# Tonz24/restir-embree

Measured on AMD Instinct MI355X. Metric: Mrays/s + frames/s at 1080p, 32 candidates, 4 spatial neighbours, higher is better.
Workload: dtype f32; 1 GPU; C2: Cornell box + 1024 emissive 0.02 m quads, A=32 B=1, spatial k=4 P=1 R=30 CONSTANT MIS, temporal off, cap 20, 1920x1080; width=1920, height=1080, traversal=lockstep, frames_in_flight=3, wide_tree=668, parallelism=1 GPU

## Files before the change

### restir-embree_amd/csrc/rs_passes.h

```cpp
#pragma once
#include "rs_scene.h"
#include "rs_texture.h"

#ifndef RS_INITIAL_WAVES
#define RS_INITIAL_WAVES 5
#endif
#ifndef RS_SPATIAL_WAVES
#define RS_SPATIAL_WAVES 4
#endif
#ifndef RS_SPATIAL_WAVES_SMALL
#define RS_SPATIAL_WAVES_SMALL 5
#endif
#ifndef RS_INITIAL_WAVES_LANE
#define RS_INITIAL_WAVES_LANE 6
#endif
#ifndef RS_SPATIAL_WAVES_LANE
#define RS_SPATIAL_WAVES_LANE 5
#endif
#ifndef RS_TEMPORAL_WAVES
#define RS_TEMPORAL_WAVES 4
#endif
#ifndef RS_TEMPORAL_WAVES_LANE
#define RS_TEMPORAL_WAVES_LANE 5
#endif
#define RS_WAVES(T, lockstep, lane) (((T) & TRAV_LANE) ? (lane) : (lockstep))
#ifndef RS_RIS_BATCH
#define RS_RIS_BATCH 2
#endif
#ifndef RS_RIS_BATCH_LANE
#define RS_RIS_BATCH_LANE 1
#endif

namespace rs {

struct FrameConst {
    int m_area, m_brdf, k, spatial_passes, cap;
    float radius, min_normal_sim, max_depth_diff;
    int do_spatial, do_temporal, do_vis_pass, reject, mis;
    vec3 bg; float tnear_off, tfar_off, normal_off;
    int use_sky;
    uint32_t seed, frame;
    int W, H;
    int y0, y1;
    int gy0, gy1;
    float inv_view[9];
    float inv_view_prev[9];
    GCam cam, camp;
    const int* row_order;
    int n_order;
    int debug_reproj;
    int canon_vis;
    uint8_t* dbg;
    float* cand_w;
    float4* cand_ray;
};

struct Counters { unsigned long long rays, primary, reproj_outside; };

struct CountSlot {
    uint2* part;
    unsigned long long* outside;
    float* row_cost;
    int y0, y1;
};

__device__ __forceinline__ uint32_t wave_sum(uint32_t v) {
    for (int o = 32; o > 0; o >>= 1) v += __shfl_xor(v, o, 64);
    return v;
}
__device__ __forceinline__ uint64_t wave_clock() { return __builtin_amdgcn_s_memrealtime(); }
__device__ __forceinline__ void row_cost_add(CountSlot C, uint64_t t0, int y) {
    if (!C.row_cost) return;
    constexpr int kRows = 8;
    const int yt = __builtin_amdgcn_readfirstlane(y) + (int)(threadIdx.x & 63);
    const float w = (float)(wave_clock() - t0) * (1.0f / kRows);
    if ((threadIdx.x & 63) < kRows && yt >= C.y0 && yt < C.y1) atomicAdd(C.row_cost + yt, w);
}
__device__ __forceinline__ void count_rays(CountSlot C, uint32_t rays, uint32_t primary, uint64_t t0, int y) {
    uint32_t r = wave_sum(rays), p = wave_sum(primary);
    if ((threadIdx.x & 63) == 0)
        C.part[((size_t)blockIdx.y * gridDim.x + blockIdx.x) * (blockDim.x >> 6) + (threadIdx.x >> 6)] = make_uint2(r, p);
    row_cost_add(C, t0, y);
}

constexpr int kReduceBlocks = 128, kReduceThreads = 64;
__device__ __forceinline__ void block_sum2(unsigned long long& r, unsigned long long& p) {
    __shared__ unsigned long long sr[16], sp[16];
    for (int o = 32; o > 0; o >>= 1) { r += __shfl_xor(r, o, 64); p += __shfl_xor(p, o, 64); }
    const int w = threadIdx.x >> 6, nw = blockDim.x >> 6;
    if ((threadIdx.x & 63) == 0) { sr[w] = r; sp[w] = p; }
    __syncthreads();
    r = 0; p = 0;
    if (threadIdx.x == 0)
        for (int i = 0; i < nw; ++i) { r += sr[i]; p += sp[i]; }
}
__global__ void __launch_bounds__(kReduceThreads) k_reduce_counts(const uint2* part, size_t n, ulonglong2* partial,
                                                                  unsigned* ticket, Counters* out, Counters* tot) {
    const size_t chunk = (n + gridDim.x - 1) / gridDim.x, b = blockIdx.x * chunk, e = b + chunk < n ? b + chunk : n;
    unsigned long long r = 0, p = 0;
    for (size_t i = b + threadIdx.x; i < e; i += kReduceThreads) { uint2 v = part[i]; r += v.x; p += v.y; }
    block_sum2(r, p);
    __shared__ bool last;
    if (threadIdx.x == 0) {
        __hip_atomic_store(&partial[blockIdx.x].x, r, __ATOMIC_RELAXED, __HIP_MEMORY_SCOPE_AGENT);
        __hip_atomic_store(&partial[blockIdx.x].y, p, __ATOMIC_RELAXED, __HIP_MEMORY_SCOPE_AGENT);
        last = __hip_atomic_fetch_add(ticket, 1u, __ATOMIC_ACQ_REL, __HIP_MEMORY_SCOPE_AGENT) == gridDim.x - 1;
    }
    __syncthreads();
    if (!last) return;
    r = 0; p = 0;
    for (unsigned i = threadIdx.x; i < gridDim.x; i += kReduceThreads) {
        r += __hip_atomic_load(&partial[i].x, __ATOMIC_RELAXED, __HIP_MEMORY_SCOPE_AGENT);
        p += __hip_atomic_load(&partial[i].y, __ATOMIC_RELAXED, __HIP_MEMORY_SCOPE_AGENT);
    }
// ... 54 lines not shown
    float cI = gmax(dot(ld, sf.nrm), 0.0f);
    float cY = fabsf(dot(-ld, s.n));
    float G = cI * cY / r2;
    r.L = (s.li * eval_brdf<Call>(sf, ld)) * G;
    r.need = r.ok && test_vis && !(r.L.x == 0.0f && r.L.y == 0.0f && r.L.z == 0.0f);
    r.dir = ld;
    r.tfar = sqrtf(r2) - F.tfar_off;
    return r;
}
__device__ __forceinline__ FPre evaluate_f_pre(const FrameConst& F, const Sample& s, vec3 cam, const GElem& g,
                                               bool test_vis, bool alive) {
    return evaluate_f_pre(F, s, g.pos, g.le.x > 0 || g.le.y > 0 || g.le.z > 0, make_frame(g, cam), test_vis, alive);
}
__device__ __forceinline__ vec3 evaluate_f_post(const FPre& p, bool occ) {
    vec3 L = p.L;
    if (p.need) L = L * (float)(!occ);
    return p.ok ? L : mk(0, 0, 0);
}
template <int T>
__device__ __forceinline__ vec3 evaluate_f(const DevScene& S, const FrameConst& F, const Sample& s, vec3 pos,
                                           bool emissive, const ShadeFrame& sf, bool test_vis, bool alive,
                                           uint32_t& rays) {
    FPre p = evaluate_f_pre(F, s, pos, emissive, sf, test_vis, alive);
    bool occ = false;
    if (test_vis) {
        rays += p.need ? 1u : 0u;
        occ = trace_any<T>(S, p.need, pos, p.dir, FLT_MIN + F.tnear_off, p.tfar);
    }
    return evaluate_f_post(p, occ);
}
template <int T>
__device__ __forceinline__ vec3 evaluate_f(const DevScene& S, const FrameConst& F, const Sample& s, vec3 cam,
                                           const GElem& g, bool test_vis, bool alive, uint32_t& rays) {
    FPre p = evaluate_f_pre(F, s, cam, g, test_vis, alive);
    bool occ = false;
    if (test_vis) {
        rays += p.need ? 1u : 0u;
        occ = trace_any<T>(S, p.need, g.pos, p.dir, FLT_MIN + F.tnear_off, p.tfar);
    }
    return evaluate_f_post(p, occ);
}

__device__ __forceinline__ float m_area(const FrameConst& F, float pa, float pb) {
    if (pa == 0.0f && pb == 0.0f) return 0.0f;
    return pa / ((float)F.m_area * pa + (float)F.m_brdf * pb);
}
__device__ __forceinline__ float m_brdf(const FrameConst& F, float pb, float pa) {
    if (pa == 0.0f && pb == 0.0f) return 0.0f;
    return pb / ((float)F.m_area * pa + (float)F.m_brdf * pb);
}

template <int T>
__device__ __forceinline__ GElem gbuffer_fill_cam(const DevScene& S, const FrameConst& F, const GCam& cam,
                                                  const float* m, int x, int y, bool active) {
    vec3 dc = mk((float)x - (float)F.W / 2.0f, (float)F.H / 2.0f - (float)y, -cam.focal);
    vec3 dw = mk(m[0] * dc.x + m[3] * dc.y + m[6] * dc.z, m[1] * dc.x + m[4] * dc.y + m[7] * dc.z,
                 m[2] * dc.x + m[5] * dc.y + m[8] * dc.z);
    dw = normalize(dw);
    SurfHit h = intersect<T>(S, active, cam.pos, dw, FLT_MIN + 0.01f);
    GElem g;
    g.pos = mk(0, 0, 0); g.nrm = g.pos; g.kd = g.pos; g.ks = g.pos; g.le = g.pos;
    g.shin = 0; g.depth = 0; g.type = 0; g.inv_im = 0;
    if (h.hit) {
        MatRec mr = load_mat(S, h.mat);
        vec3 nrm = h.normal;
        if (S.texd) apply_maps(S, h, mr, nrm, false);
        g.pos = h.point; g.nrm = nrm; g.depth = length(h.point - cam.pos);
        g.type = mr.type; g.kd = mr.kd; g.ks = mr.ks; g.le = mr.le; g.shin = mr.shin;
        if (g.type == MT_PHONG || g.type == MT_DIELECTRIC) {
            vec3 V = normalize(cam.pos - g.pos);
            g.inv_im = 1.0f / calc_I_M(dot(V, g.nrm), g.shin);
        }
    } else {
        g.le = F.use_sky ? sky_texel(S, dw) : F.bg;
    }
    return g;
}
template <int T>
__device__ __forceinline__ GElem gbuffer_fill(const DevScene& S, const FrameConst& F, int x, int y, bool active) {
    return gbuffer_fill_cam<T>(S, F, F.cam, F.inv_view, x, y, active);
}

struct LightGlobal {
    const float* cdf_g;
    const int* guide_g;
    __device__ __forceinline__ explicit LightGlobal(const DevScene& S) : cdf_g(S.cdf), guide_g(S.cdf_guide) {}
    __device__ __forceinline__ float cdf(uint32_t i) const { return cdf_g[i]; }
    __device__ __forceinline__ uint32_t guide(uint32_t j) const { return (uint32_t)guide_g[j]; }
};
template <class LT>
__device__ __forceinline__ uint32_t light_index(const LT& L, uint32_t n_emis, float ksi) {
    uint32_t j = (uint32_t)(ksi * (float)kCdfGuide);
    uint32_t lo = L.guide(j), n = L.guide(j + 1) + 1u - lo;
    if (lo + n > n_emis) n = n_emis - lo;
    while (n > 0) {
        uint32_t h = n >> 1;
        if (L.cdf(lo + h) < ksi) { lo = lo + h + 1; n = n - h - 1; } else n = h;
    }
    return lo < n_emis ? lo : n_emis - 1;
}
__device__ __forceinline__ uint32_t light_index(const DevScene& S, float ksi) {
    return light_index(LightGlobal(S), S.n_emis, ksi);
}

constexpr int kLightLdsMax = 2048;
static_assert(kLightLdsMax <= 65535, "the LDS guide holds CDF indices as uint16_t");
static_assert(kLightLdsMax % 4 == 0 && kLightLdsMax / 4 == 2 * 256 && kCdfGuide == 4 * 256,
              "LightFill: a 256-thread workgroup moves the CDF as 2 and the guide as 1 16-B load per thread");
constexpr int LIGHT_LDS = 8;
struct LightLds {
    const float* cdf_l;
    const uint16_t* guide_l;
    __device__ __forceinline__ float cdf(uint32_t i) const { return cdf_l[i]; }
    __device__ __forceinline__ uint32_t guide(uint32_t j) const { return (uint32_t)guide_l[j]; }
};
struct LightFill {
    float4 c[2];
    int4 g;
    int g_end;
    __device__ __forceinline__ static float4 cdf4(const float* cdf, uint32_t i, uint32_t n) {
        if (4u * i + 4u <= n) return reinterpret_cast<const float4*>(cdf)[i];
        float4 v = make_float4(1.0f, 1.0f, 1.0f, 1.0f);
        if (4u * i < n) v.x = cdf[4u * i];
        if (4u * i + 1u < n) v.y = cdf[4u * i + 1u];
        if (4u * i + 2u < n) v.z = cdf[4u * i + 2u];
        return v;
    }
    __device__ __forceinline__ void issue(const DevScene& S, uint32_t t) {
        const uint32_t n = S.n_emis < (uint32_t)kLightLdsMax ? S.n_emis : (uint32_t)kLightLdsMax;
        c[0] = cdf4(S.cdf, t, n);
        c[1] = cdf4(S.cdf, t + 256u, n);
        g = reinterpret_cast<const int4*>(S.cdf_guide)[t];
        g_end = t == 0 ? S.cdf_guide[kCdfGuide] : 0;
    }
    __device__ __forceinline__ void commit(float* cdf_l, uint16_t* guide_l, uint32_t t) const {
        float4* c4 = reinterpret_cast<float4*>(cdf_l);
        uint2* g2 = reinterpret_cast<uint2*>(guide_l);
        c4[t] = c[0];
        c4[t + 256u] = c[1];
        g2[t] = make_uint2((uint32_t)g.x | ((uint32_t)g.y << 16), (uint32_t)g.z | ((uint32_t)g.w << 16));
        if (t == 0) guide_l[kCdfGuide] = (uint16_t)g_end;
    }
};

template <class LT>
__device__ __forceinline__ uint32_t area_pick(const LT& L, const DevScene& S, const Rng& rng, int c) {
    Rng q = rng;
    q.n = cand_slot(c);
    return light_index(L, S.n_emis, q.range(0.0f, 1.0f));
}
__device__ __forceinline__ uint32_t area_pick(const DevScene& S, const Rng& rng, int c) {
    return area_pick(LightGlobal(S), S, rng, c);
}
struct EmisRec {
    vec3 p0, p1, p2, n0, n1, n2, le;
    float pdf_area;
    __device__ __forceinline__ static EmisRec load(const float4* E) {
        const float4 a = E[0], b = E[1], c = E[2], d = E[3];
        EmisRec r;
        r.p0 = xyz(a); r.p1 = xyz(b); r.p2 = xyz(c); r.le = xyz(d);
        r.n0 = mk(b.w, c.w, d.w);
        r.n1 = r.n0; r.n2 = r.n0;
        if (__float_as_uint(a.w) >> 31) { r.n1 = xyz(E[4]); r.n2 = xyz(E[5]); }
        r.pdf_area = fabsf(a.w);
        return r;
    }
};
__device__ __forceinline__ float emis_pdf_brdf(const DevScene& S, int id) { return S.emis[8 * id + 5].w; }

template <bool Call = false>
__device__ __forceinline__ Sample area_sample_at(const DevScene& S, const FrameConst& F, vec3 pos, const ShadeFrame& sf,
                                                 Rng& rng, uint32_t idx, float& W_out, float& mis_out) {
    const EmisRec E = EmisRec::load(S.emis + 8 * idx);
    float r1 = rng.range(0, 1), r2 = rng.range(0, 1);
    float sr = sqrtf(r1);
    float bx = 1.0f - sr, by = sr * (1.0f - r2), bz = sr * r2;
    vec3 pt = (E.p0 * bx + E.p1 * by) + E.p2 * bz;
    vec3 nn = normalize((E.n0 * bx + E.n1 * by) + E.n2 * bz);
    float pdf_area = E.pdf_area;
    vec3 ld = pt - pos;
    float r2s = dot(ld, ld);
    ld = normalize(ld);
    float cY = gmax(dot(-ld, nn), 0.0f);
    float amf = cY / r2s;
    float pba = phong_pdf<Call>(sf, ld) * amf;
    mis_out = m_area(F, pdf_area, pba);
    W_out = 1.0f / pdf_area;
    return Sample{pt, nn, E.le};
}
template <class LT>
__device__ __forceinline__ Sample area_sample(const LT& L, const DevScene& S, const FrameConst& F, vec3 pos,
                                              const ShadeFrame& sf, Rng& rng, float& W_out, float& mis_out) {
    const uint32_t idx = light_index(L, S.n_emis, rng.range(0.0f, 1.0f));
    return area_sample_at(S, F, pos, sf, rng, idx, W_out, mis_out);
}

template <int T>
__device__ __forceinline__ Sample brdf_sample(const DevScene& S, const FrameConst& F, vec3 pos, const ShadeFrame& sf,
                                              bool alive, Rng& rng, float& W_out, float& mis_out, uint32_t& rays) {
    float pdf;
    vec3 wi = sample_brdf(sf, rng, pdf);
    vec3 org = pos + sf.nrm * F.normal_off;
    rays += alive ? 1u : 0u;
    SurfHit h = intersect<T | TRAV_LANE>(S, alive, org, wi, FLT_MIN + F.tnear_off);
    W_out = 0.0f; mis_out = 0.0f;
    if (h.hit) {
        MatRec mr = load_mat(S, h.mat);
        if (mr.le.x + mr.le.y + mr.le.z > 0) {
            vec3 hn = h.normal;
            if (S.texd) apply_maps(S, h, mr, hn, true);
            vec3 ld = h.point - pos;
            float r2s = dot(ld, ld);
            ld = normalize(ld);
            float cY = gmax(dot(-ld, hn), 0.0f);
            float amf = cY / r2s;
            float pdf_area = emis_pdf_brdf(S, h.emis_id);
            float bpa = pdf * amf;
            W_out = 1.0f / bpa;
            mis_out = m_brdf(F, bpa, pdf_area);
            return Sample{h.point, hn, mr.le};
        }
    }
    return smp_invalid();
}

struct FrameSlot {
    float4* base;
    int t, n;
    __device__ __forceinline__ void store(const ShadeFrame& s) const {
        base[t] = f4(s.nrm, s.pf);
        base[n + t] = f4(s.wr, s.omp);
        base[2 * n + t] = f4(s.kd_pi, s.shin);
        base[3 * n + t] = f4(s.ks_im, s.a);
        base[4 * n + t] = make_float4(s.maxD, s.maxS, __int_as_float(s.type), 0.0f);
    }
    __device__ __forceinline__ ShadeFrame load() const {
        asm volatile("" ::: "memory");
        const float4 a = base[t], b = base[n + t], c = base[2 * n + t], d = base[3 * n + t], e = base[4 * n + t];
        ShadeFrame s;
        s.nrm = xyz(a); s.pf = a.w; s.wr = xyz(b); s.omp = b.w; s.kd_pi = xyz(c); s.shin = c.w;
        s.ks_im = xyz(d); s.a = d.w; s.maxD = e.x; s.maxS = e.y; s.type = __float_as_int(e.z);
        return s;
    }
};

template <int T, int kB>
__device__ __forceinline__ void area_batch(const DevScene& S, const FrameConst& F, vec3 pos, const ShadeFrame& sf,
                                           Rng& rng, int c0, int c_end, bool alive, bool tv, const uint32_t* pick,
                                           float* w_out, uint32_t& rays) {
    float wu[kB], wo[kB];
    bool act[kB], okb[kB], occ[kB];
    vec3 dir[kB];
    float tf[kB];
    const float inv_ma = 1.0f / (float)F.m_area;
#pragma unroll
    for (int k = 0; k < kB; ++k) {
        float Wc, mis;
        rng.n = cand_slot(c0 + k) + 1u;
        const Sample s = area_sample_at(S, F, pos, sf, rng, pick[k], Wc, mis);
        const FPre p = evaluate_f_pre(F, s, pos, false, sf, tv, alive && c0 + k < c_end);
        const float ph = length(p.L);
        const float m = F.m_brdf > 0 ? mis : inv_ma;
        wu[k] = m * ph * Wc;
        wo[k] = m * 0.0f * Wc;
        act[k] = p.need; okb[k] = p.ok; dir[k] = p.dir; tf[k] = p.tfar; occ[k] = false;
        rays += act[k] ? 1u : 0u;
    }
    if (tv) trace_any_multi<T, kB>(S, act, pos, dir, FLT_MIN + F.tnear_off, tf, occ);
#pragma unroll
    for (int k = 0; k < kB; ++k) w_out[k] = (okb[k] && !(act[k] && occ[k])) ? wu[k] : wo[k];
}
template <class LT>
__device__ __forceinline__ Sample area_redraw(const LT& L, const DevScene& S, const FrameConst& F, vec3 pos,
                                             const ShadeFrame& sf, Rng& rng, int c, bool tv, vec3& f) {
    float Wc, mis;
    rng.n = cand_slot(c);
    const Sample s = area_sample(L, S, F, pos, sf, rng, Wc, mis);
    f = evaluate_f_pre(F, s, pos, false, sf, tv, true).L;
    return s;
}
__device__ __forceinline__ Sample area_redraw(const DevScene& S, const FrameConst& F, vec3 pos, const ShadeFrame& sf,
                                             Rng& rng, int c, bool tv, vec3& f) {
    return area_redraw(LightGlobal(S), S, F, pos, sf, rng, c, tv, f);
}

template <int T, class LT>
__device__ __forceinline__ Res initial_ris(const LT& L, const DevScene& S, const FrameConst& F, vec3 pos, bool emissive,
                                           FrameSlot fs, uint32_t pix, bool in_pass, vec3& f_sel, uint32_t& rays) {
    f_sel = mk(0, 0, 0);
    Res r = res_empty();
    const bool alive = in_pass && !emissive && S.n_emis > 0;
    if (__ballot(alive) == 0) return r;
    Rng rng; rng.init(F.seed, F.frame, PASS_INITIAL, pix);
    const bool tv = !F.do_vis_pass;
    constexpr int kB = trav_lane(T) ? RS_RIS_BATCH_LANE : RS_RIS_BATCH;
    float best_phat = 0.0f;
    if (F.m_area > 0) {
        int sel = -1;
        uint32_t pick[kB];
#pragma unroll
        for (int k = 0; k < kB; ++k) pick[k] = area_pick(L, S, rng, k);
        for (int c0 = 0; c0 < F.m_area; c0 += kB) {
            float w[kB];
            uint32_t next[kB];
#pragma unroll
            for (int k = 0; k < kB; ++k) next[k] = area_pick(L, S, rng, c0 + kB + k);
            area_batch<T, kB>(S, F, pos, fs.load(), rng, c0, F.m_area, alive, tv, pick, w, rays);
#pragma unroll
            for (int k = 0; k < kB; ++k) pick[k] = next[k];
#pragma unroll
            for (int k = 0; k < kB; ++k) {
                if (c0 + k < F.m_area) {
                    rng.n = cand_slot(c0 + k) + 3u;
                    if (alive && res_add_w(r, w[k], 0, rng)) sel = c0 + k;
                }
            }
        }
        if (sel >= 0) {
            const Sample s = area_redraw(L, S, F, pos, fs.load(), rng, sel, tv, f_sel);
            best_phat = length(f_sel);
            r.p = s.p; r.n = s.n; r.li = s.li;
        }
    }
    if (F.m_brdf > 0) {
        float inv_mb = 1.0f / (float)F.m_brdf;
        for (int i = 0; i < F.m_brdf; ++i) {
            float Wc, mis;
            rng.n = cand_slot(F.m_area + i);
            const ShadeFrame sf = fs.load();
            Sample s = brdf_sample<T>(S, F, pos, sf, alive, rng, Wc, mis, rays);
            vec3 f = evaluate_f<T>(S, F, s, pos, false, sf, tv, alive, rays);
            float ph = length(f);
            float w = F.m_area > 0 ? mis * ph * Wc : inv_mb * ph * Wc;
            rng.n = cand_slot(F.m_area + i) + 3u;
            if (alive && res_add(r, s, w, 0, rng)) { best_phat = ph; f_sel = f; }
        }
    }
    if (!alive) { f_sel = mk(0, 0, 0); return res_empty(); }
    r.conf = F.m_area + F.m_brdf;
    float ph = smp_valid(smp_of(r)) ? best_phat : 0.0f;
    r.W = ph > 0.0f ? 1.0f / ph * r.wsum : 0.0f;
    res_cap(r, F.cap);
    return r;
}

__device__ __forceinline__ vec3 shade_px(const Res& r, vec3 f, vec3 le) {
    vec3 px = r.wsum > 0.0f ? f * r.W : le;
    return sanitize(px);
}
__device__ __forceinline__ void store_rgb(float* fb, size_t p, vec3 c) {
    fb[3 * p] = c.x; fb[3 * p + 1] = c.y; fb[3 * p + 2] = c.z;
}

struct TileQ { uint32_t* ctr; uint32_t n; };
__device__ __forceinline__ uint32_t q_pull(const TileQ& Q) {
    uint32_t t = 0u;
    if ((threadIdx.x & 63) == 0) t = atomicAdd(Q.ctr, 1u);
    return (uint32_t)__builtin_amdgcn_readfirstlane((int)t);
}
__device__ __forceinline__ void q_exit(const TileQ& Q) {
    if ((threadIdx.x & 63) != 0) return;
    const uint32_t waves = gridDim.x * gridDim.y * (blockDim.x >> 6);
    if (__hip_atomic_fetch_add(Q.ctr + 1, 1u, __ATOMIC_ACQ_REL, __HIP_MEMORY_SCOPE_AGENT) == waves - 1) {
        __hip_atomic_store(Q.ctr, 0u, __ATOMIC_RELAXED, __HIP_MEMORY_SCOPE_AGENT);
        __hip_atomic_store(Q.ctr + 1, 0u, __ATOMIC_RELAXED, __HIP_MEMORY_SCOPE_AGENT);
    }
}
__device__ __forceinline__ bool pixel_of_q(const FrameConst& F, int ya, int yb, uint32_t t, int& x, int& y) {
    const int W = F.W, gx = (W + 15) / 16, gy = (yb - ya + 15) / 16;
    const int q = (int)(t >> 2), w = (int)(t & 3u);
    const int bx = q % gx;
    int by = q / gx;
    if (F.row_order && ya == 0 && yb == F.H && F.n_order == gy) by = order_row(F.row_order, (uint32_t)by);
    const int lane = threadIdx.x & 63;
    x = bx * 16 + (w & 1) * 8 + (lane & 7);
    y = ya + by * 16 + (w >> 1) * 8 + (lane >> 3);
    const bool in = x < W && y < yb;
    x = x < W ? x : W - 1;
    y = y < yb ? y : yb - 1;
    return in;
}
__device__ __forceinline__ void count_store(CountSlot C, uint32_t rays, uint32_t primary) {
    const uint32_t r = wave_sum(rays), p = wave_sum(primary);
    if ((threadIdx.x & 63) == 0)
        C.part[((size_t)blockIdx.y * gridDim.x + blockIdx.x) * (blockDim.x >> 6) + (threadIdx.x >> 6)] = make_uint2(r, p);
}

template <int T, class LT>
__device__ __forceinline__ void initial_px(const LT& L, const DevScene& S, const FrameConst& F, const GElem& g,
                                           const ResBuf& Rw, float* fb, int fuse_shade, const FrameSlot& fs, int x, int y,
                                           bool in, uint32_t& rays) {
    const size_t p = (size_t)y * F.W + x;
    const bool ris = in && y >= F.y0 && y < F.y1;
    vec3 f;
    Res r = initial_ris<T>(L, S, F, g.pos, any_pos(g.le), fs, (uint32_t)p, ris, f, rays);
    if (ris) {
        Rw.store(p, r);
        if (fuse_shade) store_rgb(fb, p, shade_px(r, f, g.le));
    }
}
template <int T>
__global__ void __launch_bounds__(256, RS_WAVES(T, RS_INITIAL_WAVES, RS_INITIAL_WAVES_LANE)) k_gbuffer_initial(DevScene S, FrameConst F, GBuf G,
                                                                            ResBuf Rw, float* fb, int fuse_shade,
                                                                            CountSlot C) {
    constexpr int TT = T & ~LIGHT_LDS;
    const uint64_t t0 = wave_clock();
    if ((blockIdx.x | blockIdx.y | threadIdx.x) == 0) *C.outside = 0ull;
    int x, y;
    uint32_t rays = 0;
// ... 1028 lines not shown
```

### restir-embree_amd/csrc/rs_scene.h

```cpp
#pragma once
#include "rs_device.h"
#include "rs_lockstep.h"

namespace rs {

struct DevScene {
    const float4* nodes;
    const float4* tris;
    const float4* tri_nrm;
    const float4* mats;
    const float4* emis;
    const float* cdf;
    const int* cdf_guide;
    uint32_t n_nodes, n_tris, n_emis, n_mats;
    const float4* tri_uv;
    const float4* tri_tan;
    const uint8_t* tex;
    const int4* texd;
    int sky;
    const uint4* wnodes;
    const float4* wtris;
    uint32_t n_wnodes;
    const uint8_t* ebucket;
    vec3 ecen;
    float box_eps;
};
constexpr int kCdfGuide = 1024;

enum Trav : int { TRAV_LOCKSTEP = 0, TRAV_LANE = 1, TRAV_WIDE = 2 };
constexpr bool trav_lane(int T) { return (T & TRAV_LANE) != 0; }
constexpr bool trav_wide(int T) { return (T & TRAV_WIDE) != 0; }

__device__ __forceinline__ bool tri_test(float4 A, float4 B, float4 C, vec3 o, vec3 d, float tnear,
                                         float tfar, float& t_out, float& u_out, float& v_out) {
    vec3 v0 = xyz(A), e1 = xyz(B), e2 = xyz(C);
    vec3 p = cross(d, e2);
    float det = dot(e1, p);
    if (det == 0.0f) return false;
    float inv = 1.0f / det;
    vec3 sv = o - v0;
    float u = dot(sv, p) * inv;
    if (!(u >= 0.0f && u <= 1.0f)) return false;
    vec3 q = cross(sv, e1);
    float v = dot(d, q) * inv;
    if (!(v >= 0.0f && u + v <= 1.0f)) return false;
    float t = dot(e2, q) * inv;
    if (!(t >= tnear && t <= tfar)) return false;
    t_out = t; u_out = u; v_out = v;
    return true;
}

__device__ __forceinline__ bool tri_test_nb(float4 A, float4 B, float4 C, vec3 o, vec3 d, float tnear, float tfar,
                                            float& t, float& u, float& v) {
    vec3 v0 = xyz(A), e1 = xyz(B), e2 = xyz(C);
    vec3 p = cross(d, e2);
    float det = dot(e1, p);
    float inv = 1.0f / det;
    vec3 sv = o - v0;
    u = dot(sv, p) * inv;
    vec3 q = cross(sv, e1);
    v = dot(d, q) * inv;
    t = dot(e2, q) * inv;
    const bool ok_u = u >= 0.0f && u <= 1.0f, ok_v = v >= 0.0f && u + v <= 1.0f, ok_t = t >= tnear && t <= tfar;
    return (det != 0.0f) & ok_u & ok_v & ok_t;
}

__device__ __forceinline__ bool box_test(float4 a, float4 b, vec3 o, vec3 inv, float tnear, float tfar) {
    float tx0 = (a.x - o.x) * inv.x, tx1 = (b.x - o.x) * inv.x;
    float ty0 = (a.y - o.y) * inv.y, ty1 = (b.y - o.y) * inv.y;
    float tz0 = (a.z - o.z) * inv.z, tz1 = (b.z - o.z) * inv.z;
    float t0 = fmaxf(fmaxf(fmaxf(tnear, fminf(tx0, tx1)), fminf(ty0, ty1)), fminf(tz0, tz1));
    float t1 = fminf(fminf(fminf(tfar, fmaxf(tx0, tx1)), fmaxf(ty0, ty1)), fmaxf(tz0, tz1));
    return t0 * (1.0f - 4.0f * FLT_EPSILON) <= t1 * (1.0f + 4.0f * FLT_EPSILON);
}

__device__ __forceinline__ bool box_test_m(float4 a, float4 b, vec3 olo, vec3 ohi, vec3 inv, float tnear, float tfar) {
    float tx0 = (a.x - olo.x) * inv.x, tx1 = (b.x - ohi.x) * inv.x;
    float ty0 = (a.y - olo.y) * inv.y, ty1 = (b.y - ohi.y) * inv.y;
    float tz0 = (a.z - olo.z) * inv.z, tz1 = (b.z - ohi.z) * inv.z;
    float t0 = fmaxf(fmaxf(fmaxf(tnear, fminf(tx0, tx1)), fminf(ty0, ty1)), fminf(tz0, tz1));
    float t1 = fminf(fminf(fminf(tfar, fmaxf(tx0, tx1)), fmaxf(ty0, ty1)), fmaxf(tz0, tz1));
    return t0 * (1.0f - 4.0f * FLT_EPSILON) <= t1 * (1.0f + 4.0f * FLT_EPSILON);
}
struct MarginO { vec3 lo, hi; };
__device__ __forceinline__ MarginO margin_origins(const DevScene& S, vec3 o) {
// ... 291 lines not shown
    Hit h; h.t = tfar; h.u = 0; h.v = 0; h.prim = -1;
    if (!Wide) {
        closest_lane_from(S, active ? 0u : 0xffffffffu, o, d, inv, tnear, h);
        return h;
    }
    uint32_t occ = 0u, lost = 0u;
    wide_walk<false>(S, active, o, d, inv, tnear, tfar, h, occ, lost);
    return h;
}


__device__ __forceinline__ uint32_t wave_min_full(uint32_t v) {
    const int I = (int)0xffffffff;
    v = min(v, (uint32_t)__builtin_amdgcn_update_dpp(I, (int)v, 0xB1, 0xF, 0xF, false));
    v = min(v, (uint32_t)__builtin_amdgcn_update_dpp(I, (int)v, 0x4E, 0xF, 0xF, false));
    v = min(v, (uint32_t)__builtin_amdgcn_update_dpp(I, (int)v, 0x141, 0xF, 0xF, false));
    v = min(v, (uint32_t)__builtin_amdgcn_update_dpp(I, (int)v, 0x140, 0xF, 0xF, false));
    v = min(v, (uint32_t)__builtin_amdgcn_update_dpp(I, (int)v, 0x142, 0xA, 0xF, false));
    v = min(v, (uint32_t)__builtin_amdgcn_update_dpp(I, (int)v, 0x143, 0xC, 0xF, false));
    return (uint32_t)__builtin_amdgcn_readlane((int)v, 63);
}
__device__ __forceinline__ uint32_t wave_min_partial(uint32_t v) {
    uint32_t m = 0xffffffffu;
    uint64_t act = __ballot(1);
    while (act) {
        int lane = __builtin_ctzll(act);
        act &= act - 1;
        uint32_t x = (uint32_t)__builtin_amdgcn_readlane((int)v, lane);
        m = x < m ? x : m;
    }
    return m;
}

__device__ __forceinline__ uint32_t wave_min(bool full, uint32_t v) {
    return full ? wave_min_full(v) : wave_min_partial(v);
}
template <int K>
__device__ __forceinline__ uint32_t lane_min(const uint32_t* cur) {
    uint32_t lm = cur[0];
#pragma unroll
    for (int k = 1; k < K; ++k) lm = cur[k] < lm ? cur[k] : lm;
    return lm;
}
__device__ __forceinline__ uint32_t lockstep_step(bool leaf, bool descended, bool survivor, uint32_t m, uint32_t skip,
                                                 uint32_t lane_min_v) {
    const uint32_t next = lockstep_next(leaf, __ballot(descended) != 0, __ballot(survivor) != 0, m, skip);
    if (!leaf || next != kLockstepReduce) return next;
    return wave_min(__ballot(1) == ~0ull, lane_min_v);
}

__device__ __forceinline__ float walk_bound(float x) { return __builtin_canonicalizef(x); }
__device__ __forceinline__ bool box_test_walk(float4 a, float4 b, vec3 o, vec3 inv, float tnear_c, float tfar_c) {
#if defined(__HIP_DEVICE_COMPILE__)
    float tx0 = (a.x - o.x) * inv.x, tx1 = (b.x - o.x) * inv.x;
    float ty0 = (a.y - o.y) * inv.y, ty1 = (b.y - o.y) * inv.y;
    float tz0 = (a.z - o.z) * inv.z, tz1 = (b.z - o.z) * inv.z;
    float t0, t1;
    asm("v_max_f32 %0, %1, %2" : "=v"(t0) : "v"(tnear_c), "v"(fminf(tx0, tx1)));
    asm("v_max3_f32 %0, %1, %2, %3" : "=v"(t0) : "v"(t0), "v"(fminf(ty0, ty1)), "v"(fminf(tz0, tz1)));
    asm("v_min_f32 %0, %1, %2" : "=v"(t1) : "v"(tfar_c), "v"(fmaxf(tx0, tx1)));
    asm("v_min3_f32 %0, %1, %2, %3" : "=v"(t1) : "v"(t1), "v"(fmaxf(ty0, ty1)), "v"(fmaxf(tz0, tz1)));
    return t0 * (1.0f - 4.0f * FLT_EPSILON) <= t1 * (1.0f + 4.0f * FLT_EPSILON);
#else
    return box_test(a, b, o, inv, tnear_c, tfar_c);
#endif
}

__device__ __forceinline__ uint32_t walk_vgpr(uint32_t x) {
#if defined(__HIP_DEVICE_COMPILE__)
    asm("" : "+v"(x));
#endif
    return x;
}
__device__ __forceinline__ bool lockstep_enter(uint32_t& cur, uint32_t m, uint32_t down, uint32_t skip, float4 a, float4 b,
                                               vec3 o, vec3 inv, float tnear_c, float tfar_c) {
    bool h = false;
    if (cur == m) {
        h = box_test_walk(a, b, o, inv, tnear_c, tfar_c);
        cur = h ? down : skip;
    }
    return h;
}

template <int K>
__device__ __forceinline__ void occluded_wave_multi(const DevScene& S, const bool* active, vec3 o, const vec3* d,
                                                    float tnear, const float* tfar, bool* occ) {
    vec3 inv[K];
    uint32_t cur[K];
    float tfar_c[K];
    const float tnear_c = walk_bound(tnear);
    bool live = false;
#pragma unroll
    for (int k = 0; k < K; ++k) {
        inv[k] = mk(1.0f / d[k].x, 1.0f / d[k].y, 1.0f / d[k].z);
        cur[k] = active[k] ? 0u : kLockstepDone;
        tfar_c[k] = walk_bound(tfar[k]);
        live |= active[k];
        occ[k] = false;
    }
    const uint32_t n = S.n_nodes;
    uint32_t occb = 0u;
    uint32_t m = lockstep_first(__ballot(live) != 0);
    while (m < n) {
        float4 a, b;
        node_load(S.nodes, m, a, b);
        const uint32_t skip = (uint32_t)__float_as_int(a.w);
        const int leaf = __float_as_int(b.w);
        if (leaf >= 0) {
            uint32_t hbb = 0u;
#pragma unroll
            for (int k = 0; k < K; ++k)
                hbb |= (cur[k] == m && box_test_walk(a, b, o, inv[k], tnear_c, tfar_c[k])) ? (1u << k) : 0u;
            const int first = leaf >> 3, cnt = (leaf & 7) + 1;
            for (int j = 0; j < cnt; ++j) {
                const uint32_t want = hbb & ~occb;
                if (__ballot(want != 0u) == 0) break;
                const uint32_t tri = 3u * (uint32_t)(first + j);
                const float4 T0 = sload(S.tris, tri), T1 = sload(S.tris, tri + 1), T2 = sload(S.tris, tri + 2);
#pragma unroll
                for (int k = 0; k < K; ++k) {
                    if (__ballot((want >> k) & 1u) != 0) {
                        float t, u, v;
                        const bool hit = tri_test_nb(T0, T1, T2, o, d[k], tnear, tfar[k], t, u, v);
                        occb |= (((want >> k) & 1u) && hit) ? (1u << k) : 0u;
                    }
                }
            }
            bool survivor = false;
#pragma unroll
            for (int k = 0; k < K; ++k) {
                const bool on = cur[k] == m, ended = ((hbb & occb) >> k) & 1u;
                cur[k] = on ? (ended ? kLockstepDone : skip) : cur[k];
                survivor |= on & !ended;
            }
            m = lockstep_step(true, false, survivor, m, skip, lane_min<K>(cur));
        } else {
            const uint32_t down_v = walk_vgpr(m + 1u), skip_v = walk_vgpr(skip);
            bool desc = false;
#pragma unroll
            for (int k = 0; k < K; ++k)
                desc |= lockstep_enter(cur[k], m, down_v, skip_v, a, b, o, inv[k], tnear_c, tfar_c[k]);
            m = lockstep_step(false, desc, false, m, skip, 0u);
        }
    }
#pragma unroll
    for (int k = 0; k < K; ++k) occ[k] = (occb >> k) & 1u;
}
__device__ __forceinline__ bool occluded_wave(const DevScene& S, bool active, vec3 o, vec3 d, float tnear, float tfar) {
    vec3 inv = mk(1.0f / d.x, 1.0f / d.y, 1.0f / d.z);
    const float tnear_c = walk_bound(tnear), tfar_c = walk_bound(tfar);
    const uint32_t n = S.n_nodes;
    uint32_t i = active ? 0u : kLockstepDone;
    uint32_t occ = 0u;
    uint32_t m = lockstep_first(__ballot(active) != 0);
    while (m < n) {
        float4 a, b;
        node_load(S.nodes, m, a, b);
        const uint32_t skip = (uint32_t)__float_as_int(a.w);
        const int leaf = __float_as_int(b.w);
        if (leaf >= 0) {
            const bool at = i == m;
            const bool hb = at && box_test_walk(a, b, o, inv, tnear_c, tfar_c);
            const int first = leaf >> 3, cnt = (leaf & 7) + 1;
            for (int k = 0; k < cnt; ++k) {
                const bool want = hb && occ == 0u;
                if (__ballot(want) == 0) break;
                const uint32_t tri = 3u * (uint32_t)(first + k);
                float t, u, v;
                const bool hit = tri_test_nb(sload(S.tris, tri), sload(S.tris, tri + 1), sload(S.tris, tri + 2), o, d,
                                             tnear, tfar, t, u, v);
                occ = (want && hit) ? 1u : occ;
            }
            const bool ended = hb && occ;
            i = at ? (ended ? kLockstepDone : skip) : i;
            m = lockstep_step(true, false, at && !ended, m, skip, i);
        } else {
            const bool desc = lockstep_enter(i, m, m + 1u, skip, a, b, o, inv, tnear_c, tfar_c);
            m = lockstep_step(false, desc, false, m, skip, 0u);
        }
    }
    return occ != 0u;
}
__device__ __forceinline__ Hit closest_wave(const DevScene& S, bool active, vec3 o, vec3 d, float tnear, float tfar) {
    vec3 inv = mk(1.0f / d.x, 1.0f / d.y, 1.0f / d.z);
    const MarginO mo = margin_origins(S, o);
    Hit h; h.t = tfar; h.u = 0; h.v = 0; h.prim = -1;
    const uint32_t n = S.n_nodes;
    uint32_t i = active ? 0u : kLockstepDone;
    uint32_t m = lockstep_first(__ballot(active) != 0);
    while (m < n) {
        float4 a, b;
        node_load(S.nodes, m, a, b);
        const uint32_t skip = (uint32_t)__float_as_int(a.w);
        const int leaf = __float_as_int(b.w);
        if (leaf >= 0) {
            const bool at = i == m;
            const bool hb = at && box_test_m(a, b, mo.lo, mo.hi, inv, tnear, h.t);
            if (__ballot(hb) != 0) {
                const int first = leaf >> 3, cnt = (leaf & 7) + 1;
                for (int k = 0; k < cnt; ++k) {
                    const uint32_t tri = 3u * (uint32_t)(first + k);
                    const float4 T0 = sload(S.tris, tri);
                    float t, u, v;
                    const bool hit = hb & tri_test_nb(T0, sload(S.tris, tri + 1), sload(S.tris, tri + 2), o, d, tnear,
                                                       h.t, t, u, v);
                    const int prim = __float_as_int(T0.w);
                    const bool better = hit && (h.prim < 0 || t < h.t || (t == h.t && prim < h.prim));
                    h.t = better ? t : h.t; h.u = better ? u : h.u; h.v = better ? v : h.v;
                    h.prim = better ? prim : h.prim;
                }
            }
            i = at ? skip : i;
            m = lockstep_next(true, false, true, m, skip);
        } else {
            bool hb = false;
            if (i == m) {
                hb = box_test_m(a, b, mo.lo, mo.hi, inv, tnear, h.t);
                i = hb ? m + 1u : skip;
            }
            m = lockstep_next(false, __ballot(hb) != 0, false, m, skip);
        }
    }
    return h;
}

template <int T, int K>
__device__ __forceinline__ void trace_any_multi(const DevScene& S, const bool* active, vec3 o, const vec3* d,
                                                float tnear, const float* tfar, bool* occ) {
    if (!trav_lane(T)) {
        occluded_wave_multi<K>(S, active, o, d, tnear, tfar, occ);
    } else {
#pragma unroll
        for (int k = 0; k < K; ++k) occ[k] = occluded_lane<trav_wide(T)>(S, active[k], o, d[k], tnear, tfar[k]);
    }
}
template <int T>
__device__ __forceinline__ bool trace_any(const DevScene& S, bool active, vec3 o, vec3 d, float tnear, float tfar) {
    if (!trav_lane(T)) return occluded_wave(S, active, o, d, tnear, tfar);
    return occluded_lane<trav_wide(T)>(S, active, o, d, tnear, tfar);
}
template <int T>
__device__ __forceinline__ Hit trace_closest(const DevScene& S, bool active, vec3 o, vec3 d, float tnear, float tfar) {
    if (!trav_lane(T)) return closest_wave(S, active, o, d, tnear, tfar);
    return closest_lane<trav_wide(T)>(S, active, o, d, tnear, tfar);
}

struct MatRec { vec3 kd; float shin; vec3 ks; int type; vec3 le; };
constexpr int kMatStride = 4;
__device__ __forceinline__ MatRec load_mat(const DevScene& S, uint32_t m) {
    float4 a = S.mats[kMatStride * m], b = S.mats[kMatStride * m + 1], c = S.mats[kMatStride * m + 2];
    return MatRec{xyz(a), a.w, xyz(b), __float_as_int(b.w), xyz(c)};
}
__device__ __forceinline__ int4 load_maps(const DevScene& S, uint32_t m) {
    float4 q = S.mats[kMatStride * m + 3];
    return make_int4(__float_as_int(q.x), __float_as_int(q.y), __float_as_int(q.z), __float_as_int(q.w));
}

struct SurfHit { bool hit; vec3 point, normal; uint32_t mat; int emis_id; int prim; float u, v; };
template <int T>
__device__ __forceinline__ SurfHit intersect(const DevScene& S, bool active, vec3 o, vec3 d, float tnear) {
    SurfHit r; r.hit = false; r.mat = 0; r.emis_id = -1; r.point = mk(0, 0, 0); r.normal = mk(0, 0, 0);
    r.prim = -1; r.u = 0.0f; r.v = 0.0f;
    Hit h = trace_closest<T>(S, active, o, d, tnear, FLT_MAX);
    if (h.prim < 0) return r;
    const float4* N = S.tri_nrm + 3 * h.prim;
    float4 n0 = N[0], n1 = N[1], n2 = N[2];
    float w = 1.0f - h.u - h.v;
    vec3 n = (xyz(n0) * w + xyz(n1) * h.u) + xyz(n2) * h.v;
    n = normalize(n);
    if (dot(-d, n) <= 0.0f) n = n * -1.0f;
    r.hit = true; r.normal = n; r.point = o + d * h.t;
    r.mat = (uint32_t)__float_as_int(n0.w); r.emis_id = __float_as_int(n1.w);
    r.prim = h.prim; r.u = h.u; r.v = h.v;
    return r;
}

}
```

Measured before the change: 872.0 frames/s.

## Batch three area candidates per lockstep traversal and ride BRDF shadow ray along

For lockstep traversal, initial RIS now batches three area candidates per wave-wide shadow traversal instead of two. When the candidate count is not a multiple of the batch, the first BRDF candidate's shadow ray fills the last slot of the final batch, so the lockstep BVH walk is shared. The change also skips pick-ahead prefetch when lights are in LDS, uses bitmask occlusion outputs, and uses the clamped walk bounds in triangle tests. It reduces the number of full BVH walks per pixel, at the cost of more registers per batch and extra control-flow complexity.

```diff
diff --git a/restir-embree_amd/csrc/rs_passes.h b/restir-embree_amd/csrc/rs_passes.h
--- a/restir-embree_amd/csrc/rs_passes.h
+++ b/restir-embree_amd/csrc/rs_passes.h
@@ -30,6 +30,9 @@
 #ifndef RS_RIS_BATCH_LANE
 #define RS_RIS_BATCH_LANE 1
 #endif
+#ifndef RS_RIS_BATCH_PIXEL
+#define RS_RIS_BATCH_PIXEL 3
+#endif
 
 namespace rs {
 
@@ -250,6 +253,7 @@
 }
 
 struct LightGlobal {
+    static constexpr bool kLds = false;
     const float* cdf_g;
     const int* guide_g;
     __device__ __forceinline__ explicit LightGlobal(const DevScene& S) : cdf_g(S.cdf), guide_g(S.cdf_guide) {}
@@ -277,6 +281,7 @@
               "LightFill: a 256-thread workgroup moves the CDF as 2 and the guide as 1 16-B load per thread");
 constexpr int LIGHT_LDS = 8;
 struct LightLds {
+    static constexpr bool kLds = true;
     const float* cdf_l;
     const uint16_t* guide_l;
     __device__ __forceinline__ float cdf(uint32_t i) const { return cdf_l[i]; }
@@ -438,6 +443,42 @@
 #pragma unroll
     for (int k = 0; k < kB; ++k) w_out[k] = (okb[k] && !(act[k] && occ[k])) ? wu[k] : wo[k];
 }
+template <int T, int kA, int kR>
+__device__ __forceinline__ void area_batch_px(const DevScene& S, const FrameConst& F, vec3 pos, const ShadeFrame& sf,
+                                              Rng& rng, int c0, int c_end, bool alive, bool tv, const uint32_t* pick,
+                                              float* w_out, uint32_t& rays, const FPre& ride, bool& ride_occ) {
+    float wu[kA], wo[kA];
+    uint32_t need = 0u, ok = 0u;
+    vec3 dir[kA + kR];
+    float tf[kA + kR];
+    const float inv_ma = 1.0f / (float)F.m_area;
+#pragma unroll
+    for (int k = 0; k < kA; ++k) {
+        float Wc, mis;
+        rng.n = cand_slot(c0 + k) + 1u;
+        const Sample s = area_sample_at(S, F, pos, sf, rng, pick[k], Wc, mis);
+        const FPre p = evaluate_f_pre(F, s, pos, false, sf, tv, alive && c0 + k < c_end);
+        const float ph = length(p.L);
+        const float m = F.m_brdf > 0 ? mis : inv_ma;
+        wu[k] = m * ph * Wc;
+        wo[k] = m * 0.0f * Wc;
+        need |= p.need ? 1u << k : 0u;
+        ok |= p.ok ? 1u << k : 0u;
+        dir[k] = p.dir; tf[k] = p.tfar;
+        rays += p.need ? 1u : 0u;
+        __builtin_amdgcn_sched_barrier(0);
+    }
+    if (kR) {
+        need |= ride.need ? 1u << kA : 0u;
+        dir[kA] = ride.dir; tf[kA] = ride.tfar;
+    }
+    uint32_t occ = 0u;
+    if (tv) occ = trace_any_bits<T, kA + kR>(S, need, pos, dir, FLT_MIN + F.tnear_off, tf);
+    const uint32_t lit = ok & ~occ;
+#pragma unroll
+    for (int k = 0; k < kA; ++k) w_out[k] = ((lit >> k) & 1u) ? wu[k] : wo[k];
+    ride_occ = (occ >> kA) & 1u;
+}
 template <class LT>
 __device__ __forceinline__ Sample area_redraw(const LT& L, const DevScene& S, const FrameConst& F, vec3 pos,
                                              const ShadeFrame& sf, Rng& rng, int c, bool tv, vec3& f) {
@@ -461,21 +502,41 @@
     if (__ballot(alive) == 0) return r;
     Rng rng; rng.init(F.seed, F.frame, PASS_INITIAL, pix);
     const bool tv = !F.do_vis_pass;
-    constexpr int kB = trav_lane(T) ? RS_RIS_BATCH_LANE : RS_RIS_BATCH;
+    constexpr bool kLane = trav_lane(T);
+    constexpr int kB = kLane ? RS_RIS_BATCH_LANE : RS_RIS_BATCH_PIXEL;
+    constexpr bool kAhead = kLane || !LT::kLds;
+    const bool ride = !kLane && tv && F.m_brdf > 0 && F.m_area % kB != 0;
+    const int a_loop = ride ? F.m_area - F.m_area % kB : F.m_area;
+    const FPre no_ride{};
+    bool ride_occ = false;
     float best_phat = 0.0f;
     if (F.m_area > 0) {
         int sel = -1;
         uint32_t pick[kB];
-#pragma unroll
-        for (int k = 0; k < kB; ++k) pick[k] = area_pick(L, S, rng, k);
-        for (int c0 = 0; c0 < F.m_area; c0 += kB) {
+        if constexpr (kAhead) {
+#pragma unroll
+            for (int k = 0; k < kB; ++k) pick[k] = area_pick(L, S, rng, k);
+        }
+        for (int c = 0; !kLane && !tv && c < F.m_area; ++c) {
+            if constexpr (!kLane) {
+                float w;
+                pick[0] = area_pick(L, S, rng, c);
+                area_batch_px<T, 1, 0>(S, F, pos, fs.load(), rng, c, F.m_area, alive, tv, pick, &w, rays, no_ride, ride_occ);
+                rng.n = cand_slot(c) + 3u;
+                if (alive && res_add_w(r, w, 0, rng)) sel = c;
+            }
+        }
+        for (int c0 = 0; (kLane || tv) && c0 < a_loop; c0 += kB) {
             float w[kB];
             uint32_t next[kB];
 #pragma unroll
-            for (int k = 0; k < kB; ++k) next[k] = area_pick(L, S, rng, c0 + kB + k);
-            area_batch<T, kB>(S, F, pos, fs.load(), rng, c0, F.m_area, alive, tv, pick, w, rays);
-#pragma unroll
-            for (int k = 0; k < kB; ++k) pick[k] = next[k];
+            for (int k = 0; k < kB; ++k) (kAhead ? next[k] : pick[k]) = area_pick(L, S, rng, c0 + (kAhead ? kB : 0) + k);
+            if constexpr (kLane) area_batch<T, kB>(S, F, pos, fs.load(), rng, c0, F.m_area, alive, tv, pick, w, rays);
+            else area_batch_px<T, kB, 0>(S, F, pos, fs.load(), rng, c0, F.m_area, alive, tv, pick, w, rays, no_ride, ride_occ);
+            if constexpr (kAhead) {
+#pragma unroll
+                for (int k = 0; k < kB; ++k) pick[k] = next[k];
+            }
 #pragma unroll
             for (int k = 0; k < kB; ++k) {
                 if (c0 + k < F.m_area) {
@@ -484,7 +545,41 @@
                 }
             }
         }
-        if (sel >= 0) {
+        if constexpr (!kLane) {
+            if (ride) {
+                float Wc, mis, w[kB - 1];
+                const ShadeFrame sf = fs.load();
+                rng.n = cand_slot(F.m_area);
+                const Sample s = brdf_sample<T>(S, F, pos, sf, alive, rng, Wc, mis, rays);
+                const FPre p = evaluate_f_pre(F, s, pos, false, sf, tv, alive);
+                rays += p.need ? 1u : 0u;
+                if constexpr (!kAhead) {
+#pragma unroll
+                    for (int k = 0; k < kB - 1; ++k) pick[k] = area_pick(L, S, rng, a_loop + k);
+                }
+                area_batch_px<T, kB - 1, 1>(S, F, pos, sf, rng, a_loop, F.m_area, alive, tv, pick, w, rays, p, ride_occ);
+#pragma unroll
+                for (int k = 0; k < kB - 1; ++k) {
+                    if (a_loop + k < F.m_area) {
+                        rng.n = cand_slot(a_loop + k) + 3u;
+                        if (alive && res_add_w(r, w[k], 0, rng)) sel = a_loop + k;
+                    }
+                }
+                if (sel >= 0) {
+                    const Sample sa = area_redraw(L, S, F, pos, fs.load(), rng, sel, tv, f_sel);
+                    best_phat = length(f_sel);
+                    r.p = sa.p; r.n = sa.n; r.li = sa.li;
+                }
+                const vec3 f = evaluate_f_post(p, ride_occ);
+                const float ph = length(f);
+                rng.n = cand_slot(F.m_area) + 3u;
+                if (alive && res_add(r, s, mis * ph * Wc, 0, rng)) { best_phat = ph; f_sel = f; }
+            } else if (sel >= 0) {
+                const Sample s = area_redraw(L, S, F, pos, fs.load(), rng, sel, tv, f_sel);
+                best_phat = length(f_sel);
+                r.p = s.p; r.n = s.n; r.li = s.li;
+            }
+        } else if (sel >= 0) {
             const Sample s = area_redraw(L, S, F, pos, fs.load(), rng, sel, tv, f_sel);
             best_phat = length(f_sel);
             r.p = s.p; r.n = s.n; r.li = s.li;
@@ -492,7 +587,7 @@
     }
     if (F.m_brdf > 0) {
         float inv_mb = 1.0f / (float)F.m_brdf;
-        for (int i = 0; i < F.m_brdf; ++i) {
+        for (int i = ride ? 1 : 0; i < F.m_brdf; ++i) {
             float Wc, mis;
             rng.n = cand_slot(F.m_area + i);
             const ShadeFrame sf = fs.load();
diff --git a/restir-embree_amd/csrc/rs_scene.h b/restir-embree_amd/csrc/rs_scene.h
--- a/restir-embree_amd/csrc/rs_scene.h
+++ b/restir-embree_amd/csrc/rs_scene.h
@@ -1,6 +1,7 @@
 #pragma once
 #include "rs_device.h"
 #include "rs_lockstep.h"
+#include <type_traits>
 
 namespace rs {
 
@@ -458,9 +459,11 @@
     return h;
 }
 
-template <int K>
-__device__ __forceinline__ void occluded_wave_multi(const DevScene& S, const bool* active, vec3 o, const vec3* d,
-                                                    float tnear, const float* tfar, bool* occ) {
+__device__ __forceinline__ bool ray_on(const bool* active, int k) { return active[k]; }
+__device__ __forceinline__ bool ray_on(uint32_t active, int k) { return (active >> k) & 1u; }
+template <int K, bool kOneBound, class A, class O>
+__device__ __forceinline__ void occluded_wave_multi(const DevScene& S, A active, vec3 o, const vec3* d, float tnear,
+                                                    const float* tfar, O& occ) {
     vec3 inv[K];
     uint32_t cur[K];
     float tfar_c[K];
@@ -469,10 +472,9 @@
 #pragma unroll
     for (int k = 0; k < K; ++k) {
         inv[k] = mk(1.0f / d[k].x, 1.0f / d[k].y, 1.0f / d[k].z);
-        cur[k] = active[k] ? 0u : kLockstepDone;
+        cur[k] = ray_on(active, k) ? 0u : kLockstepDone;
         tfar_c[k] = walk_bound(tfar[k]);
-        live |= active[k];
-        occ[k] = false;
+        live |= ray_on(active, k);
     }
     const uint32_t n = S.n_nodes;
     uint32_t occb = 0u;
@@ -497,7 +499,8 @@
                 for (int k = 0; k < K; ++k) {
                     if (__ballot((want >> k) & 1u) != 0) {
                         float t, u, v;
-                        const bool hit = tri_test_nb(T0, T1, T2, o, d[k], tnear, tfar[k], t, u, v);
+                        const bool hit = tri_test_nb(T0, T1, T2, o, d[k], kOneBound ? tnear_c : tnear,
+                                                     kOneBound ? tfar_c[k] : tfar[k], t, u, v);
                         occb |= (((want >> k) & 1u) && hit) ? (1u << k) : 0u;
                     }
                 }
@@ -519,8 +522,12 @@
             m = lockstep_step(false, desc, false, m, skip, 0u);
         }
     }
-#pragma unroll
-    for (int k = 0; k < K; ++k) occ[k] = (occb >> k) & 1u;
+    if constexpr (std::is_same_v<O, uint32_t>) {
+        occ = occb;
+    } else {
+#pragma unroll
+        for (int k = 0; k < K; ++k) occ[k] = (occb >> k) & 1u;
+    }
 }
 __device__ __forceinline__ bool occluded_wave(const DevScene& S, bool active, vec3 o, vec3 d, float tnear, float tfar) {
     vec3 inv = mk(1.0f / d.x, 1.0f / d.y, 1.0f / d.z);
@@ -604,11 +611,19 @@
 __device__ __forceinline__ void trace_any_multi(const DevScene& S, const bool* active, vec3 o, const vec3* d,
                                                 float tnear, const float* tfar, bool* occ) {
     if (!trav_lane(T)) {
-        occluded_wave_multi<K>(S, active, o, d, tnear, tfar, occ);
+        occluded_wave_multi<K, false>(S, active, o, d, tnear, tfar, occ);
     } else {
 #pragma unroll
         for (int k = 0; k < K; ++k) occ[k] = occluded_lane<trav_wide(T)>(S, active[k], o, d[k], tnear, tfar[k]);
     }
+}
+template <int T, int K>
+__device__ __forceinline__ uint32_t trace_any_bits(const DevScene& S, uint32_t active, vec3 o, const vec3* d, float tnear,
+                                                   const float* tfar) {
+    static_assert(!trav_lane(T), "the per-lane kinds trace one ray after the other (trace_any_multi)");
+    uint32_t occ = 0u;
+    occluded_wave_multi<K, true>(S, active, o, d, tnear, tfar, occ);
+    return occ;
 }
 template <int T>
 __device__ __forceinline__ bool trace_any(const DevScene& S, bool active, vec3 o, vec3 d, float tnear, float tfar) {
```

Result: faster. 896.4 frames/s, median of 6 (+2.8%).
